# NVlabs/STEP

Hardware: NVIDIA H100
Metric: clips/sec (T=32,224x224) STEP max_iter=3 (higher is better)
Workload: dtype f16

## Files before the change

step_b200/csrc/conv_umma.cu:

```cuda
#include <cuda.h>
#include <stdlib.h>
#include <string.h>

#include "common.cuh"
#include "umma_ptx.cuh"

namespace step {

constexpr int kBM = 128;
constexpr int kMaxBN = 256;
constexpr int kStages = 8;
constexpr int kThreads = 384;
constexpr int kConsumers = 256;
constexpr int kCopyThreads = 96;
constexpr int kPersistMaxKBlocks = 100;
constexpr int kBookBytes = 2 * kStages * 8 + 2 * 8 + 2 * 2 * kMaxBN * 4;
constexpr int kProducerRegs = 40, kConsumerRegs = 232;

#define STEP_CONV_TILES(X)                                                                                         \
  X(64, 32) X(64, 64) X(64, 128) X(64, 144) X(64, 152) X(64, 176) X(64, 192) X(64, 208) X(64, 224) X(64, 256)      \
  X(32, 64) X(32, 128) X(32, 144) X(32, 152) X(32, 160) X(32, 208) X(32, 224)                                      \
  X(16, 64)

__host__ __device__ constexpr int staging_pitch(int BN) { return ((BN / 8 + 1) | 1) * 16; }

struct ConvGeom {
  int mode;
  int taps, KT, KH, KW, PT, PH, PW;
  int kblocks_per_tap;
  int BN, n_tiles;
  int n_stages;
  int n_splits, split[2], ld_extra[2], coff_extra[2];
  __half* y_extra[2];
  int Cout, out_ld, out_coff, res_ld, res_coff, relu;
  int OT, OH, OW, Nimg;
  long long M;
  int tiles;
  int bw, bh, bt, tiles_w, tiles_h, tiles_t;
  int a_bytes;
};

__device__ __forceinline__ long long tile_row_pixel(const ConvGeom& g, int m_tile, int row) {
  if (g.mode == STEP_A_BOX) {
    int r = m_tile;
    const int bw0 = (r % g.tiles_w) * g.bw; r /= g.tiles_w;
    const int bh0 = (r % g.tiles_h) * g.bh; r /= g.tiles_h;
    const int bt0 = (r % g.tiles_t) * g.bt; const int bn = r / g.tiles_t;
    const int dw = row % g.bw, rr = row / g.bw;
    const int dh = rr % g.bh, dt = rr / g.bh;
    const int ow = bw0 + dw, oh = bh0 + dh, ot = bt0 + dt;
    if (dt < g.bt && ow < g.OW && oh < g.OH && ot < g.OT) return (((long long)bn * g.OT + ot) * g.OH + oh) * g.OW + ow;
    return -1;
  }
  const long long m = (long long)m_tile * kBM + row;
  return m < g.M ? m : -1;
}

__device__ __forceinline__ bool mbar_try_wait(uint64_t* bar, uint32_t parity) {
  uint32_t done;
  asm volatile("{\n\t.reg .pred p;\n\tmbarrier.try_wait.parity.shared::cta.b64 p, [%1], %2;\n\tselp.u32 %0, 1, 0, p;\n\t}"
               : "=r"(done) : "r"(smem_u32(bar)), "r"(parity) : "memory");
  return done != 0;
}

template <int BK, int BN>
__global__ void __launch_bounds__(kThreads, 1)
conv_umma_kernel(const __grid_constant__ CUtensorMap map_a, const __grid_constant__ CUtensorMap map_b, ConvGeom g,
                 const float* __restrict__ scale, const float* __restrict__ shift, const __half* __restrict__ residual,
                 __half* __restrict__ y) {
  static_assert(BN % 8 == 0 && BN <= kMaxBN, "wgmma N is a multiple of 8, at most 256");
  constexpr bool kRealloc = BN > 128;
  constexpr bool kBulkOut = BN > 128;
  constexpr int kABytes = kBM * BK * 2;
  constexpr int kBBytes = BN * BK * 2;
  extern __shared__ __align__(1024) uint8_t smem_raw[];
  uint64_t* full_bar = (uint64_t*)smem_raw;
  uint64_t* empty_bar = full_bar + kStages;
  uint64_t* out_full = empty_bar + kStages;
  uint64_t* out_empty = out_full + 1;
  float* s_consts = (float*)(out_empty + 1);
  uint8_t* smem = (uint8_t*)(((uintptr_t)smem_raw + kBookBytes + 1023) & ~(uintptr_t)1023);
  uint8_t* sA = smem;
  uint8_t* sB = smem + g.n_stages * kABytes;
  uint8_t* stg = smem + g.n_stages * (kABytes + kBBytes);
  constexpr int pitch = staging_pitch(BN);

  const int warp = threadIdx.x >> 5, lane = threadIdx.x & 31;
  const int num_kb = g.taps * g.kblocks_per_tap;

  if (threadIdx.x == 0) {
    prefetch_tensormap(&map_a);
    prefetch_tensormap(&map_b);
    for (int s = 0; s < kStages; ++s) { mbar_init(&full_bar[s], 1); mbar_init(&empty_bar[s], 2); }
    mbar_init(out_full, kConsumers / 32);
    mbar_init(out_empty, kCopyThreads / 32);
    fence_barrier_init();
  }
  auto stage_consts = [&](int n_tile, int buf, int t, int nthr) {
    float* s_scale = s_consts + buf * 2 * kMaxBN;
    float* s_shift = s_scale + kMaxBN;
    for (int i = t; i < BN; i += nthr) {
      const int c = n_tile * BN + i;
      s_scale[i] = (scale && c < g.Cout) ? scale[c] : 1.0f;
      s_shift[i] = (shift && c < g.Cout) ? shift[c] : 0.0f;
    }
  };
  if (threadIdx.x < 128) stage_consts(blockIdx.x % g.n_tiles, 0, threadIdx.x, 128);
  __syncthreads();

  if (warp < 4) {
    if constexpr (kRealloc) setmaxnreg_dec<kProducerRegs>();
    if (warp == 0) {
      if (elect_one()) {
        const uint32_t tx_bytes = (uint32_t)(g.a_bytes + kBBytes);
        int stage = 0; uint32_t phase = 0;
        for (int tile = blockIdx.x; tile < g.tiles; tile += gridDim.x) {
          const int m_tile = tile / g.n_tiles, n0 = (tile - m_tile * g.n_tiles) * BN;
          long long m0 = (long long)m_tile * kBM;
          int bn = 0, bt0 = 0, bh0 = 0, bw0 = 0;
          if (g.mode == STEP_A_BOX) {
            int r = m_tile;
            bw0 = (r % g.tiles_w) * g.bw; r /= g.tiles_w;
            bh0 = (r % g.tiles_h) * g.bh; r /= g.tiles_h;
            bt0 = (r % g.tiles_t) * g.bt; bn = r / g.tiles_t;
          }
          int iw = 0, ih = 0, it = 0, in_ = 0;
          if (g.mode == STEP_A_IM2COL) {
            long long r = m0;
            iw = (int)(r % g.OW); r /= g.OW;
            ih = (int)(r % g.OH); r /= g.OH;
            it = (int)(r % g.OT); in_ = (int)(r / g.OT);
            iw -= g.PW; ih -= g.PH; it -= g.PT;
          }
          int kw = 0, kh = 0, kt = 0;
          for (int tap = 0; tap < g.taps; ++tap) {
            for (int kc = 0; kc < g.kblocks_per_tap; ++kc) {
              mbar_wait(&empty_bar[stage], phase ^ 1);
              mbar_expect_tx(&full_bar[stage], tx_bytes);
              const int c0 = kc * BK;
              uint8_t* a_dst = sA + stage * kABytes;
              if (g.mode == STEP_A_LINEAR) {
                tma_load_2d(&map_a, &full_bar[stage], a_dst, c0, (int)m0);
              } else if (g.mode == STEP_A_BOX) {
                tma_load_5d(&map_a, &full_bar[stage], a_dst, c0, bw0 + kw - g.PW, bh0 + kh - g.PH, bt0 + kt - g.PT, bn);
              } else {
                tma_load_im2col_5d(&map_a, &full_bar[stage], a_dst, c0, iw, ih, it, in_, (uint16_t)kw, (uint16_t)kh,
                                   (uint16_t)kt);
              }
              tma_load_3d(&map_b, &full_bar[stage], sB + stage * kBBytes, c0, tap, n0);
              if (++stage == g.n_stages) { stage = 0; phase ^= 1; }
            }
            if (++kw == g.KW) { kw = 0; if (++kh == g.KH) { kh = 0; ++kt; } }
          }
        }
      }
    } else {
      const int ct = threadIdx.x - 32;
      int i_tile = 0;
      for (int tile = blockIdx.x; tile < g.tiles; tile += gridDim.x, ++i_tile) {
        const int m_tile = tile / g.n_tiles, n0 = (tile - m_tile * g.n_tiles) * BN;
        if (tile + (int)gridDim.x < g.tiles) stage_consts((tile + gridDim.x) % g.n_tiles, (i_tile + 1) & 1, ct, kCopyThreads);
        while (!mbar_try_wait(out_full, i_tile & 1)) __nanosleep(128);
        if constexpr (!kBulkOut) {
          constexpr int cpr = BN / 8;
          constexpr int kUnroll = 4;
          for (int i0 = ct; i0 < kBM * cpr; i0 += kUnroll * kCopyThreads) {
            uint4 val[kUnroll];
#pragma unroll
            for (int u = 0; u < kUnroll; ++u) {
              const int i = i0 + u * kCopyThreads, rr = i / cpr, ch = i - rr * cpr;
              if (i < kBM * cpr) val[u] = *reinterpret_cast<const uint4*>(stg + (size_t)rr * pitch + ch * 16);
            }
#pragma unroll
            for (int u = 0; u < kUnroll; ++u) {
              const int i = i0 + u * kCopyThreads, rr = i / cpr, ch = i - rr * cpr;
              const int col = n0 + ch * 8;
              if (i >= kBM * cpr || col >= g.Cout) continue;
              const long long rp = tile_row_pixel(g, m_tile, rr);
              if (rp < 0) continue;
              __half* dst = y + (size_t)rp * g.out_ld + g.out_coff + col;
              if (g.n_splits > 0 && col >= g.split[0]) {
                const int d = (g.n_splits > 1 && col >= g.split[1]) ? 1 : 0;
                dst = g.y_extra[d] + (size_t)rp * g.ld_extra[d] + g.coff_extra[d] + (col - g.split[d]);
              }
              *reinterpret_cast<uint4*>(dst) = val[u];
            }
          }
          __syncwarp();
          if (lane == 0) mbar_arrive(out_empty);
          continue;
        }
        const int end = min(n0 + BN, g.Cout);
        for (int rr = ct; rr < kBM; rr += kCopyThreads) {
          const long long rp = tile_row_pixel(g, m_tile, rr);
          if (rp < 0) continue;
          for (int col = n0; col < end;) {
            __half* dst = y + (size_t)rp * g.out_ld + g.out_coff + col;
            int next = end;
            if (g.n_splits > 0) {
              if (col >= g.split[0]) {
                const int d = (g.n_splits > 1 && col >= g.split[1]) ? 1 : 0;
                dst = g.y_extra[d] + (size_t)rp * g.ld_extra[d] + g.coff_extra[d] + (col - g.split[d]);
                if (d == 0 && g.n_splits > 1) next = min(end, g.split[1]);
              } else {
                next = min(end, g.split[0]);
              }
            }
            bulk_store(dst, stg + (size_t)rr * pitch + (col - n0) * 2, (uint32_t)(next - col) * 2);
            col = next;
          }
        }
        bulk_commit();
        bulk_wait_read<0>();
        __syncwarp();
        if (lane == 0) mbar_arrive(out_empty);
      }
    }
  } else {
    if constexpr (kRealloc) setmaxnreg_inc<kConsumerRegs>();
    const int wg = (warp >> 2) - 1;
    const int ct = threadIdx.x - 128;
    const uint64_t hi = desc_hi_kmajor<BK>();
    const uint64_t a_lo0 = desc_lo(sA + wg * 64 * BK * 2), b_lo0 = desc_lo(sB);
    const int wrow = wg * 64 + (warp & 3) * 16 + (lane >> 2);
    float acc[BN / 2];
    int stage = 0; uint32_t phase = 0;
    int i_tile = 0;
    for (int tile = blockIdx.x; tile < g.tiles; tile += gridDim.x, ++i_tile) {
      const int m_tile = tile / g.n_tiles, n0 = (tile - m_tile * g.n_tiles) * BN;
#pragma unroll
      for (int i = 0; i < BN / 2; ++i) acc[i] = 0.0f;
      int prev = -1;
      for (int kb = 0; kb < num_kb; ++kb) {
        mbar_wait(&full_bar[stage], phase);
        const uint64_t a_lo = a_lo0 + (uint64_t)(stage * (kABytes >> 4)), b_lo = b_lo0 + (uint64_t)(stage * (kBBytes >> 4));
        wg_fence();
#pragma unroll
        for (int k = 0; k < BK / 16; ++k)
          wgmma_f16<BN>(acc, hi | (a_lo + 2 * k), hi | (b_lo + 2 * k), 1u);
        wg_commit();
        wg_wait<1>();
        if (prev >= 0 && ct % 128 == 0) mbar_arrive(&empty_bar[prev]);
        prev = stage;
        if (++stage == g.n_stages) { stage = 0; phase ^= 1; }
      }
      wg_wait<0>();
      if (ct % 128 == 0) mbar_arrive(&empty_bar[prev]);
      mbar_wait(out_empty, (i_tile & 1) ^ 1);
      const float* s_scale = s_consts + (i_tile & 1) * 2 * kMaxBN;
      const float* s_shift = s_scale + kMaxBN;
#pragma unroll
      for (int i = 0; i < 2; ++i) {
        const int row = wrow + 8 * i;
        const long long pix = residual ? tile_row_pixel(g, m_tile, row) : -1;
        const __half* rrow = pix >= 0 ? residual + (size_t)pix * g.res_ld + g.res_coff + n0 : nullptr;
        uint8_t* srow = stg + (size_t)row * pitch;
#pragma unroll
        for (int j = 0; j < BN / 8; ++j) {
          const int col = 8 * j + 2 * (lane & 3);
          float f0 = fmaf(acc[4 * j + 2 * i], s_scale[col], s_shift[col]);
          float f1 = fmaf(acc[4 * j + 2 * i + 1], s_scale[col + 1], s_shift[col + 1]);
          if (rrow && n0 + col < g.Cout) {
            const float2 rf = __half22float2(*reinterpret_cast<const __half2*>(rrow + col));
            f0 += rf.x; f1 += rf.y;
          }
          if (g.relu) { f0 = fmaxf(f0, 0.0f); f1 = fmaxf(f1, 0.0f); }
          *reinterpret_cast<__half2*>(srow + col * 2) = __floats2half2_rn(f0, f1);
        }
      }
      if constexpr (kBulkOut) fence_proxy_async();
      __syncwarp();
      if (lane == 0) mbar_arrive(out_full);
    }
  }
}

template <int BK>
__global__ void __launch_bounds__(32) tma_dump_kernel(const __grid_constant__ CUtensorMap map_a, ConvGeom g, int m_tile,
                                                      int kt, int kh, int kw, int c0, uint8_t* __restrict__ out) {
  constexpr int kABytes = kBM * BK * 2;
  extern __shared__ __align__(1024) uint8_t smem_raw[];
  uint8_t* smem = (uint8_t*)(((uintptr_t)smem_raw + 1023) & ~(uintptr_t)1023);
  __shared__ uint64_t bar;
  for (int i = threadIdx.x; i < kABytes / 4; i += 32) ((uint32_t*)smem)[i] = 0xFFFFFFFFu;
  if (threadIdx.x == 0) { mbar_init(&bar, 1); fence_barrier_init(); }
  fence_proxy_async();
  __syncwarp();
  if (threadIdx.x == 0) {
    long long m0 = (long long)m_tile * kBM;
    mbar_expect_tx(&bar, (uint32_t)g.a_bytes);
    if (g.mode == STEP_A_LINEAR) {
      tma_load_2d(&map_a, &bar, smem, c0, (int)m0);
    } else if (g.mode == STEP_A_BOX) {
      int r = m_tile;
      int bw0 = (r % g.tiles_w) * g.bw; r /= g.tiles_w;
      int bh0 = (r % g.tiles_h) * g.bh; r /= g.tiles_h;
      int bt0 = (r % g.tiles_t) * g.bt; int bn = r / g.tiles_t;
      tma_load_5d(&map_a, &bar, smem, c0, bw0 + kw - g.PW, bh0 + kh - g.PH, bt0 + kt - g.PT, bn);
    } else {
      long long r = m0;
      int iw = (int)(r % g.OW); r /= g.OW;
      int ih = (int)(r % g.OH); r /= g.OH;
      int it = (int)(r % g.OT); int in_ = (int)(r / g.OT);
      tma_load_im2col_5d(&map_a, &bar, smem, c0, iw - g.PW, ih - g.PH, it - g.PT, in_, (uint16_t)kw, (uint16_t)kh, (uint16_t)kt);
    }
  }
  mbar_wait(&bar, 0);
  __syncwarp();
  for (int i = threadIdx.x; i < kABytes / 4; i += 32) ((uint32_t*)out)[i] = ((uint32_t*)smem)[i];
}

static int pick_bk(int Cin) {
  if (Cin <= 16) return 16;
  const int k64 = (Cin + 63) / 64 * 64, k32 = (Cin + 31) / 32 * 32;
  return k32 < k64 ? 32 : 64;
}

struct ConvTile {
  int BK, BN;
  void (*kernel)(CUtensorMap, CUtensorMap, ConvGeom, const float*, const float*, const __half*, __half*);
};
static const ConvTile kTiles[] = {
#define STEP_TILE_ENTRY(bk, bn) {bk, bn, conv_umma_kernel<bk, bn>},
    STEP_CONV_TILES(STEP_TILE_ENTRY)
#undef STEP_TILE_ENTRY
};
constexpr int kNumTiles = (int)(sizeof(kTiles) / sizeof(kTiles[0]));

static int pick_tile(int BK, int Cout) {
  int best = -1; long best_pad = 0, best_n = 0;
  for (int i = 0; i < kNumTiles; ++i) {
    if (kTiles[i].BK != BK) continue;
    const long n = (Cout + kTiles[i].BN - 1) / kTiles[i].BN, pad = n * kTiles[i].BN - Cout;
    if (best < 0 || pad < best_pad || (pad == best_pad && n < best_n)) { best = i; best_pad = pad; best_n = n; }
  }
  return best;
}

static void pick_box(int OW, int OH, int OT, int* bw, int* bh, int* bt) {
  double best = -1;
  for (int w = 1; w <= OW && w <= kBM; ++w)
    for (int h = 1; h <= OH && w * h <= kBM; ++h) {
      int t = kBM / (w * h);
      if (t > OT) t = OT;
      if (t < 1) continue;
      double eff = ((double)OW / (((OW + w - 1) / w) * w)) * ((double)OH / (((OH + h - 1) / h) * h)) *
                   ((double)OT / (((OT + t - 1) / t) * t)) * ((double)(w * h * t) / kBM);
      if (eff > best + 1e-9) { best = eff; *bw = w; *bh = h; *bt = t; }
    }
}

static std::atomic<int> g_two_ctas[kNumTiles];
static std::atomic<unsigned long long> g_attr_seen[kNumTiles];

static int two_ctas_fit(int t, size_t smem, bool* two) {
  int v = g_two_ctas[t].load(std::memory_order_relaxed);
  if (v == 0) {
    cudaError_t e = cudaFuncSetAttribute(kTiles[t].kernel, cudaFuncAttributeMaxDynamicSharedMemorySize, 227 * 1024);
    int n = 0;
    if (e == cudaSuccess) e = cudaOccupancyMaxActiveBlocksPerMultiprocessor(&n, kTiles[t].kernel, kThreads, smem);
    if (e != cudaSuccess) { cudaGetLastError(); return fail((int)e, "conv3d(f16): occupancy query: %s", cudaGetErrorString(e)); }
    v = n >= 2 ? 2 : 1;
    g_two_ctas[t].store(v, std::memory_order_relaxed);
  }
  *two = v == 2;
  return 0;
}

static std::atomic<int> g_sm_count[64];

static int sm_count(int* n) {
  int dev = 0;
  cudaError_t e = cudaGetDevice(&dev);
  if (e != cudaSuccess) { cudaGetLastError(); return fail((int)e, "conv3d(f16): cudaGetDevice: %s", cudaGetErrorString(e)); }
  int v = g_sm_count[dev & 63].load(std::memory_order_relaxed);
  if (v == 0) {
    e = cudaDeviceGetAttribute(&v, cudaDevAttrMultiProcessorCount, dev);
    if (e != cudaSuccess) { cudaGetLastError(); return fail((int)e, "conv3d(f16): SM count: %s", cudaGetErrorString(e)); }
    g_sm_count[dev & 63].store(v, std::memory_order_relaxed);
  }
  *n = v;
  return 0;
}

struct ConvPlan {
  CUtensorMap map_a, map_b;
  ConvGeom g;
  int BK;
  int tile;
  size_t smem_bytes;
  dim3 grid;
};

static int build_plan(const step_conv_params* p, ConvPlan* pl) {
  STEP_CHECK_ARG(p->ST == 1 && p->SH == 1 && p->SW == 1, "conv3d(f16): stride must be 1 (use the s2d stem)");
  STEP_CHECK_ARG(p->Cin % 8 == 0 && p->in_ld % 8 == 0 && p->w_ld % 8 == 0 && p->w_ld >= p->Cin,
                 "conv3d(f16): Cin=%d in_ld=%d w_ld=%d must be multiples of 8", p->Cin, p->in_ld, p->w_ld);
  STEP_CHECK_ARG(p->Cout % 8 == 0 && p->out_ld % 8 == 0 && p->out_coff % 8 == 0, "conv3d(f16): Cout/out_ld/out_coff %% 8");
  STEP_CHECK_ARG(!p->residual || (p->res_ld % 8 == 0 && p->res_coff % 8 == 0), "conv3d(f16): res_ld/res_coff %% 8");
  STEP_CHECK_ARG((((uintptr_t)p->x | (uintptr_t)p->w | (uintptr_t)p->y | (uintptr_t)p->residual) & 15) == 0,
                 "conv3d(f16): pointers must be 16-byte aligned");
  ConvGeom& g = pl->g;
  memset(&g, 0, sizeof(g));
  const int taps = p->KT * p->KH * p->KW;
  const bool is_1x1 = taps == 1 && p->PT == 0 && p->PH == 0 && p->PW == 0 && p->OT == p->T && p->OH == p->H && p->OW == p->W;
  int mode = p->a_mode;
  if (mode == STEP_A_AUTO) mode = is_1x1 ? STEP_A_LINEAR : STEP_A_BOX;
  STEP_CHECK_ARG(mode == STEP_A_LINEAR || mode == STEP_A_BOX || mode == STEP_A_IM2COL, "conv3d(f16): bad a_mode %d", p->a_mode);
  STEP_CHECK_ARG(mode != STEP_A_LINEAR || is_1x1, "conv3d(f16): LINEAR mode needs a 1x1x1 unpadded filter");
  g.mode = mode;
  g.taps = taps; g.KT = p->KT; g.KH = p->KH; g.KW = p->KW; g.PT = p->PT; g.PH = p->PH; g.PW = p->PW;
  pl->BK = pick_bk(p->Cin);
  const int BK = pl->BK;
  g.kblocks_per_tap = (p->Cin + BK - 1) / BK;
  pl->tile = pick_tile(BK, p->Cout);
  g.BN = kTiles[pl->tile].BN;
  g.n_tiles = (p->Cout + g.BN - 1) / g.BN;
  g.Cout = p->Cout; g.out_ld = p->out_ld; g.out_coff = p->out_coff; g.res_ld = p->res_ld; g.res_coff = p->res_coff;
  g.relu = p->relu;
  g.n_splits = p->n_splits;
  if (p->n_splits) {
    STEP_CHECK_ARG(p->n_splits >= 1 && p->n_splits <= 2 && !p->residual, "conv3d(f16): fused outputs need no residual, 1-2 splits");
    int prev = 0;
    for (int i = 0; i < p->n_splits; ++i) {
      STEP_CHECK_ARG(p->split[i] % 16 == 0 && p->split[i] > prev && p->split[i] < p->Cout && p->y_extra[i] &&
                     p->ld_extra[i] % 8 == 0 && p->coff_extra[i] % 8 == 0 && ((uintptr_t)p->y_extra[i] & 15) == 0,
                     "conv3d(f16): bad split %d", i);
      prev = p->split[i];
      g.split[i] = p->split[i]; g.y_extra[i] = (__half*)p->y_extra[i]; g.ld_extra[i] = p->ld_extra[i]; g.coff_extra[i] = p->coff_extra[i];
    }
    STEP_CHECK_ARG(p->out_ld >= p->out_coff + p->split[0], "conv3d(f16): first destination too narrow");
  }
  g.OT = p->OT; g.OH = p->OH; g.OW = p->OW; g.Nimg = p->N;
  g.M = (long long)p->N * p->OT * p->OH * p->OW;
  long long m_tiles;
  int rc;
  if (mode == STEP_A_LINEAR) {
    STEP_CHECK_ARG(g.M < (1LL << 31), "conv3d(f16): M too large");
    rc = encode_rows2d(&pl->map_a, p->x, g.M, p->Cin, p->in_ld, BK, kBM, swizzle_for(BK), CU_TENSOR_MAP_L2_PROMOTION_L2_128B,
                       "conv3d(f16): A (linear)");
    m_tiles = (g.M + kBM - 1) / kBM;
    g.a_bytes = kBM * BK * 2;
  } else {
    const ActLayout act(p->N, p->T, p->H, p->W, p->Cin, p->in_ld);
    if (mode == STEP_A_BOX) {
      pick_box(p->OW, p->OH, p->OT, &g.bw, &g.bh, &g.bt);
      g.tiles_w = (p->OW + g.bw - 1) / g.bw; g.tiles_h = (p->OH + g.bh - 1) / g.bh; g.tiles_t = (p->OT + g.bt - 1) / g.bt;
      const cuuint32_t box[5] = {(cuuint32_t)BK, (cuuint32_t)g.bw, (cuuint32_t)g.bh, (cuuint32_t)g.bt, 1};
      rc = encode_act5d(&pl->map_a, p->x, act, box, swizzle_for(BK), CU_TENSOR_MAP_L2_PROMOTION_L2_128B, "conv3d(f16): A (box)");
      m_tiles = (long long)p->N * g.tiles_t * g.tiles_h * g.tiles_w;
      g.a_bytes = g.bw * g.bh * g.bt * BK * 2;
    } else {
      const int ph_t = p->OT - p->T + p->KT - 1 - p->PT, ph_h = p->OH - p->H + p->KH - 1 - p->PH,
                ph_w = p->OW - p->W + p->KW - 1 - p->PW;
      int lower[3] = {-p->PW, -p->PH, -p->PT};
      int upper[3] = {ph_w - (p->KW - 1), ph_h - (p->KH - 1), ph_t - (p->KT - 1)};
      for (int i = 0; i < 3; ++i)
        STEP_CHECK_ARG(lower[i] >= -16 && lower[i] <= 15 && upper[i] >= -16 && upper[i] <= 15, "conv3d(f16): im2col corner range");
      rc = encode_act5d_im2col(&pl->map_a, p->x, act, lower, upper, BK, kBM, swizzle_for(BK),
                               CU_TENSOR_MAP_L2_PROMOTION_L2_128B, "conv3d(f16): A (im2col)");
      int drv = 0;
      cudaDriverGetVersion(&drv);
      if (rc == 0 && drv <= 13010 &&
          (size_t)p->N * p->T * p->H * p->W * p->in_ld * 2 < 131072)
        reinterpret_cast<uint64_t*>(&pl->map_a)[1] &= ~(1ULL << 21);
      m_tiles = (g.M + kBM - 1) / kBM;
      g.a_bytes = kBM * BK * 2;
    }
  }
  if (rc) return rc;
  if ((rc = encode_weights3d(&pl->map_b, p->w, p->Cout, taps, p->Cin, p->w_ld, BK, g.BN, swizzle_for(BK),
                             CU_TENSOR_MAP_L2_PROMOTION_L2_256B, "conv3d(f16): B")))
    return rc;
  STEP_CHECK_ARG(m_tiles * g.n_tiles < (1LL << 31), "conv3d(f16): grid too large");
  g.tiles = (int)(m_tiles * g.n_tiles);
  const long per_stage = (long)kBM * BK * 2 + (long)g.BN * BK * 2;
  const long fixed = kBookBytes + 1024 + (long)kBM * staging_pitch(g.BN);
  int st = (int)((113L * 1024 - fixed) / per_stage);
  if (st > kStages) st = kStages;
  bool two = false;
  if (st >= 3) {
    if (int rc = two_ctas_fit(pl->tile, (size_t)(fixed + st * per_stage), &two)) return rc;
  }
  if (!two) st = (int)((227L * 1024 - fixed) / per_stage);
  g.n_stages = st > kStages ? kStages : st;
  STEP_CHECK_ARG(g.n_stages >= 2, "conv3d(f16): tile does not fit shared memory");
  pl->smem_bytes = (size_t)(fixed + g.n_stages * per_stage);
  int sms = 0;
  if (int rc = sm_count(&sms)) return rc;
  const long resident = (long)sms * (two ? 2 : 1);
  const bool persist = g.taps * g.kblocks_per_tap <= kPersistMaxKBlocks && g.tiles > resident;
  pl->grid = dim3((unsigned)(persist ? resident : g.tiles));
  return 0;
}

int conv3d_umma_launch(const step_conv_params* p, step_stream_t stream) {
  ConvPlan pl;
  if (int rc = build_plan(p, &pl)) return rc;
  const ConvTile& t = kTiles[pl.tile];
  if (int rc = allow_dynamic_smem(t.kernel, g_attr_seen[pl.tile], 227 * 1024, "conv_umma_kernel")) return rc;
  return launch_tc("conv_umma_kernel", t.kernel, pl.grid, kThreads, pl.smem_bytes, cu(stream), pl.map_a, pl.map_b, pl.g,
                   p->scale, p->shift, (const __half*)p->residual, (__half*)p->y);
}

}

using namespace step;

extern "C" int step_debug_tma_tile(const step_conv_params* p, int m_tile, int kt, int kh, int kw, int c0, void* out,
                                   int* bk_out, int* box_out , step_stream_t stream) {
  ConvPlan pl;
  if (int rc = build_plan(p, &pl)) return rc;
  if (bk_out) *bk_out = pl.BK;
  if (box_out) { box_out[0] = pl.g.bw; box_out[1] = pl.g.bh; box_out[2] = pl.g.bt; }
  size_t smem = 1024 + (size_t)kBM * pl.BK * 2;
  if (pl.BK == 64) tma_dump_kernel<64><<<1, 32, smem, cu(stream)>>>(pl.map_a, pl.g, m_tile, kt, kh, kw, c0, (uint8_t*)out);
  else if (pl.BK == 32) tma_dump_kernel<32><<<1, 32, smem, cu(stream)>>>(pl.map_a, pl.g, m_tile, kt, kh, kw, c0, (uint8_t*)out);
  else tma_dump_kernel<16><<<1, 32, smem, cu(stream)>>>(pl.map_a, pl.g, m_tile, kt, kh, kw, c0, (uint8_t*)out);
  STEP_LAUNCH_CHECK("tma_dump_kernel");
  return 0;
}
```

Baseline: 1161.

## Load and multiply only the needed channels in the last K block

Adds narrower tail tensor maps for activations and weights so the last K block of each tap loads only the channels it needs (16, 32 or 64 wide). The consumer runs fewer wgmma K-steps for that block, using a matching descriptor and per-warpgroup offset. BK selection now weighs N-tile padding for BK 64 against BK 32, and several BK=32 tile variants are dropped. This removes zero-padding traffic and MMA work when Cin is not a multiple of BK, at the cost of extra tensor maps, more kernel parameters and more template branching.

```diff
diff --git a/step_b200/csrc/conv_umma.cu b/step_b200/csrc/conv_umma.cu
--- a/step_b200/csrc/conv_umma.cu
+++ b/step_b200/csrc/conv_umma.cu
@@ -1,6 +1,8 @@
 #include <cuda.h>
 #include <stdlib.h>
 #include <string.h>
+
+#include <type_traits>
 
 #include "common.cuh"
 #include "umma_ptx.cuh"
@@ -19,8 +21,13 @@
 
 #define STEP_CONV_TILES(X)                                                                                         \
   X(64, 32) X(64, 64) X(64, 128) X(64, 144) X(64, 152) X(64, 176) X(64, 192) X(64, 208) X(64, 224) X(64, 256)      \
-  X(32, 64) X(32, 128) X(32, 144) X(32, 152) X(32, 160) X(32, 208) X(32, 224)                                      \
+  X(32, 64) X(32, 128) X(32, 160)                                                                                  \
   X(16, 64)
+
+__host__ __device__ constexpr int tail_width(int tail, int BK) {
+  const int w = tail <= 1 ? 16 : (tail == 2 ? 32 : 64);
+  return w < BK ? w : BK;
+}
 
 __host__ __device__ constexpr int staging_pitch(int BN) { return ((BN / 8 + 1) | 1) * 16; }
 
@@ -28,6 +35,8 @@
   int mode;
   int taps, KT, KH, KW, PT, PH, PW;
   int kblocks_per_tap;
+  int tail;
+  int tail_w, a_tail_bytes;
   int BN, n_tiles;
   int n_stages;
   int n_splits, split[2], ld_extra[2], coff_extra[2];
@@ -65,7 +74,8 @@
 
 template <int BK, int BN>
 __global__ void __launch_bounds__(kThreads, 1)
-conv_umma_kernel(const __grid_constant__ CUtensorMap map_a, const __grid_constant__ CUtensorMap map_b, ConvGeom g,
+conv_umma_kernel(const __grid_constant__ CUtensorMap map_a, const __grid_constant__ CUtensorMap map_b,
+                 const __grid_constant__ CUtensorMap map_a_tail, const __grid_constant__ CUtensorMap map_b_tail, ConvGeom g,
                  const float* __restrict__ scale, const float* __restrict__ shift, const __half* __restrict__ residual,
                  __half* __restrict__ y) {
   static_assert(BN % 8 == 0 && BN <= kMaxBN, "wgmma N is a multiple of 8, at most 256");
@@ -86,11 +96,11 @@
   constexpr int pitch = staging_pitch(BN);
 
   const int warp = threadIdx.x >> 5, lane = threadIdx.x & 31;
-  const int num_kb = g.taps * g.kblocks_per_tap;
 
   if (threadIdx.x == 0) {
     prefetch_tensormap(&map_a);
     prefetch_tensormap(&map_b);
+    if (g.tail_w < BK) { prefetch_tensormap(&map_a_tail); prefetch_tensormap(&map_b_tail); }
     for (int s = 0; s < kStages; ++s) { mbar_init(&full_bar[s], 1); mbar_init(&empty_bar[s], 2); }
     mbar_init(out_full, kConsumers / 32);
     mbar_init(out_empty, kCopyThreads / 32);
@@ -113,6 +123,7 @@
     if (warp == 0) {
       if (elect_one()) {
         const uint32_t tx_bytes = (uint32_t)(g.a_bytes + kBBytes);
+        const uint32_t tx_tail = (uint32_t)(g.a_tail_bytes + BN * g.tail_w * 2);
         int stage = 0; uint32_t phase = 0;
         for (int tile = blockIdx.x; tile < g.tiles; tile += gridDim.x) {
           const int m_tile = tile / g.n_tiles, n0 = (tile - m_tile * g.n_tiles) * BN;
@@ -135,19 +146,21 @@
           int kw = 0, kh = 0, kt = 0;
           for (int tap = 0; tap < g.taps; ++tap) {
             for (int kc = 0; kc < g.kblocks_per_tap; ++kc) {
+              const bool narrow = kc == g.kblocks_per_tap - 1 && g.tail_w < BK;
+              const CUtensorMap* ma = narrow ? &map_a_tail : &map_a;
               mbar_wait(&empty_bar[stage], phase ^ 1);
-              mbar_expect_tx(&full_bar[stage], tx_bytes);
+              mbar_expect_tx(&full_bar[stage], narrow ? tx_tail : tx_bytes);
               const int c0 = kc * BK;
               uint8_t* a_dst = sA + stage * kABytes;
               if (g.mode == STEP_A_LINEAR) {
-                tma_load_2d(&map_a, &full_bar[stage], a_dst, c0, (int)m0);
+                tma_load_2d(ma, &full_bar[stage], a_dst, c0, (int)m0);
               } else if (g.mode == STEP_A_BOX) {
-                tma_load_5d(&map_a, &full_bar[stage], a_dst, c0, bw0 + kw - g.PW, bh0 + kh - g.PH, bt0 + kt - g.PT, bn);
+                tma_load_5d(ma, &full_bar[stage], a_dst, c0, bw0 + kw - g.PW, bh0 + kh - g.PH, bt0 + kt - g.PT, bn);
               } else {
-                tma_load_im2col_5d(&map_a, &full_bar[stage], a_dst, c0, iw, ih, it, in_, (uint16_t)kw, (uint16_t)kh,
+                tma_load_im2col_5d(ma, &full_bar[stage], a_dst, c0, iw, ih, it, in_, (uint16_t)kw, (uint16_t)kh,
                                    (uint16_t)kt);
               }
-              tma_load_3d(&map_b, &full_bar[stage], sB + stage * kBBytes, c0, tap, n0);
+              tma_load_3d(narrow ? &map_b_tail : &map_b, &full_bar[stage], sB + stage * kBBytes, c0, tap, n0);
               if (++stage == g.n_stages) { stage = 0; phase ^= 1; }
             }
             if (++kw == g.KW) { kw = 0; if (++kh == g.KH) { kh = 0; ++kt; } }
@@ -220,8 +233,7 @@
     if constexpr (kRealloc) setmaxnreg_inc<kConsumerRegs>();
     const int wg = (warp >> 2) - 1;
     const int ct = threadIdx.x - 128;
-    const uint64_t hi = desc_hi_kmajor<BK>();
-    const uint64_t a_lo0 = desc_lo(sA + wg * 64 * BK * 2), b_lo0 = desc_lo(sB);
+    const uint64_t a_lo0 = desc_lo(sA), b_lo0 = desc_lo(sB);
     const int wrow = wg * 64 + (warp & 3) * 16 + (lane >> 2);
     float acc[BN / 2];
     int stage = 0; uint32_t phase = 0;
@@ -231,18 +243,40 @@
 #pragma unroll
       for (int i = 0; i < BN / 2; ++i) acc[i] = 0.0f;
       int prev = -1;
-      for (int kb = 0; kb < num_kb; ++kb) {
+      auto kblock = [&](auto steps, auto width) {
+        const uint64_t hi = desc_hi_kmajor<decltype(width)::value>();
         mbar_wait(&full_bar[stage], phase);
-        const uint64_t a_lo = a_lo0 + (uint64_t)(stage * (kABytes >> 4)), b_lo = b_lo0 + (uint64_t)(stage * (kBBytes >> 4));
+        constexpr int wg_rows = (64 * decltype(width)::value * 2) >> 4;
+        const uint64_t a_lo = a_lo0 + (uint64_t)(stage * (kABytes >> 4) + wg * wg_rows);
+        const uint64_t b_lo = b_lo0 + (uint64_t)(stage * (kBBytes >> 4));
         wg_fence();
 #pragma unroll
-        for (int k = 0; k < BK / 16; ++k)
+        for (int k = 0; k < decltype(steps)::value; ++k)
           wgmma_f16<BN>(acc, hi | (a_lo + 2 * k), hi | (b_lo + 2 * k), 1u);
         wg_commit();
         wg_wait<1>();
         if (prev >= 0 && ct % 128 == 0) mbar_arrive(&empty_bar[prev]);
         prev = stage;
         if (++stage == g.n_stages) { stage = 0; phase ^= 1; }
+      };
+      using full = std::integral_constant<int, BK / 16>;
+      using bk = std::integral_constant<int, BK>;
+      for (int tap = 0; tap < g.taps; ++tap) {
+        for (int kc = 1; kc < g.kblocks_per_tap; ++kc) kblock(full(), bk());
+        switch (g.tail) {
+          case 1:
+            kblock(std::integral_constant<int, 1>(), std::integral_constant<int, tail_width(1, BK)>());
+            break;
+          case 2:
+            kblock(std::integral_constant<int, 2 < BK / 16 ? 2 : BK / 16>(), std::integral_constant<int, tail_width(2, BK)>());
+            break;
+          case 3:
+            kblock(std::integral_constant<int, 3 < BK / 16 ? 3 : BK / 16>(), std::integral_constant<int, tail_width(3, BK)>());
+            break;
+          default:
+            kblock(full(), bk());
+            break;
+        }
       }
       wg_wait<0>();
       if (ct % 128 == 0) mbar_arrive(&empty_bar[prev]);
@@ -310,15 +344,10 @@
   for (int i = threadIdx.x; i < kABytes / 4; i += 32) ((uint32_t*)out)[i] = ((uint32_t*)smem)[i];
 }
 
-static int pick_bk(int Cin) {
-  if (Cin <= 16) return 16;
-  const int k64 = (Cin + 63) / 64 * 64, k32 = (Cin + 31) / 32 * 32;
-  return k32 < k64 ? 32 : 64;
-}
-
 struct ConvTile {
   int BK, BN;
-  void (*kernel)(CUtensorMap, CUtensorMap, ConvGeom, const float*, const float*, const __half*, __half*);
+  void (*kernel)(CUtensorMap, CUtensorMap, CUtensorMap, CUtensorMap, ConvGeom, const float*, const float*, const __half*,
+                 __half*);
 };
 static const ConvTile kTiles[] = {
 #define STEP_TILE_ENTRY(bk, bn) {bk, bn, conv_umma_kernel<bk, bn>},
@@ -335,6 +364,17 @@
     if (best < 0 || pad < best_pad || (pad == best_pad && n < best_n)) { best = i; best_pad = pad; best_n = n; }
   }
   return best;
+}
+
+static int pick_tile_bk(int Cin, int Cout, int* BK) {
+  if (Cin <= 32) { *BK = Cin <= 16 ? 16 : 32; return pick_tile(*BK, Cout); }
+  const int t64 = pick_tile(64, Cout), t32 = pick_tile(32, Cout);
+  auto cost = [&](int t, long* n) { *n = (Cout + kTiles[t].BN - 1) / kTiles[t].BN; return *n * kTiles[t].BN - Cout; };
+  long n64, n32;
+  const long pad64 = cost(t64, &n64), pad32 = cost(t32, &n32);
+  const bool narrow = pad32 < pad64 || (pad32 == pad64 && n32 < n64);
+  *BK = narrow ? 32 : 64;
+  return narrow ? t32 : t64;
 }
 
 static void pick_box(int OW, int OH, int OT, int* bw, int* bh, int* bt) {
@@ -385,6 +425,7 @@
 
 struct ConvPlan {
   CUtensorMap map_a, map_b;
+  CUtensorMap map_a_tail, map_b_tail;
   ConvGeom g;
   int BK;
   int tile;
@@ -410,10 +451,12 @@
   STEP_CHECK_ARG(mode != STEP_A_LINEAR || is_1x1, "conv3d(f16): LINEAR mode needs a 1x1x1 unpadded filter");
   g.mode = mode;
   g.taps = taps; g.KT = p->KT; g.KH = p->KH; g.KW = p->KW; g.PT = p->PT; g.PH = p->PH; g.PW = p->PW;
-  pl->BK = pick_bk(p->Cin);
+  pl->tile = pick_tile_bk(p->Cin, p->Cout, &pl->BK);
   const int BK = pl->BK;
   g.kblocks_per_tap = (p->Cin + BK - 1) / BK;
-  pl->tile = pick_tile(BK, p->Cout);
+  g.tail = (p->Cin - (g.kblocks_per_tap - 1) * BK + 15) / 16;
+  g.tail_w = tail_width(g.tail, BK);
+  const int TW = g.tail_w;
   g.BN = kTiles[pl->tile].BN;
   g.n_tiles = (p->Cout + g.BN - 1) / g.BN;
   g.Cout = p->Cout; g.out_ld = p->out_ld; g.out_coff = p->out_coff; g.res_ld = p->res_ld; g.res_coff = p->res_coff;
@@ -439,8 +482,12 @@
     STEP_CHECK_ARG(g.M < (1LL << 31), "conv3d(f16): M too large");
     rc = encode_rows2d(&pl->map_a, p->x, g.M, p->Cin, p->in_ld, BK, kBM, swizzle_for(BK), CU_TENSOR_MAP_L2_PROMOTION_L2_128B,
                        "conv3d(f16): A (linear)");
+    if (rc == 0 && TW < BK)
+      rc = encode_rows2d(&pl->map_a_tail, p->x, g.M, p->Cin, p->in_ld, TW, kBM, swizzle_for(TW),
+                         CU_TENSOR_MAP_L2_PROMOTION_L2_128B, "conv3d(f16): A tail (linear)");
     m_tiles = (g.M + kBM - 1) / kBM;
     g.a_bytes = kBM * BK * 2;
+    g.a_tail_bytes = kBM * TW * 2;
   } else {
     const ActLayout act(p->N, p->T, p->H, p->W, p->Cin, p->in_ld);
     if (mode == STEP_A_BOX) {
@@ -448,8 +495,13 @@
       g.tiles_w = (p->OW + g.bw - 1) / g.bw; g.tiles_h = (p->OH + g.bh - 1) / g.bh; g.tiles_t = (p->OT + g.bt - 1) / g.bt;
       const cuuint32_t box[5] = {(cuuint32_t)BK, (cuuint32_t)g.bw, (cuuint32_t)g.bh, (cuuint32_t)g.bt, 1};
       rc = encode_act5d(&pl->map_a, p->x, act, box, swizzle_for(BK), CU_TENSOR_MAP_L2_PROMOTION_L2_128B, "conv3d(f16): A (box)");
+      const cuuint32_t box_tail[5] = {(cuuint32_t)TW, (cuuint32_t)g.bw, (cuuint32_t)g.bh, (cuuint32_t)g.bt, 1};
+      if (rc == 0 && TW < BK)
+        rc = encode_act5d(&pl->map_a_tail, p->x, act, box_tail, swizzle_for(TW), CU_TENSOR_MAP_L2_PROMOTION_L2_128B,
+                          "conv3d(f16): A tail (box)");
       m_tiles = (long long)p->N * g.tiles_t * g.tiles_h * g.tiles_w;
       g.a_bytes = g.bw * g.bh * g.bt * BK * 2;
+      g.a_tail_bytes = g.bw * g.bh * g.bt * TW * 2;
     } else {
       const int ph_t = p->OT - p->T + p->KT - 1 - p->PT, ph_h = p->OH - p->H + p->KH - 1 - p->PH,
                 ph_w = p->OW - p->W + p->KW - 1 - p->PW;
@@ -459,19 +511,33 @@
         STEP_CHECK_ARG(lower[i] >= -16 && lower[i] <= 15 && upper[i] >= -16 && upper[i] <= 15, "conv3d(f16): im2col corner range");
       rc = encode_act5d_im2col(&pl->map_a, p->x, act, lower, upper, BK, kBM, swizzle_for(BK),
                                CU_TENSOR_MAP_L2_PROMOTION_L2_128B, "conv3d(f16): A (im2col)");
+      if (rc == 0 && TW < BK)
+        rc = encode_act5d_im2col(&pl->map_a_tail, p->x, act, lower, upper, TW, kBM, swizzle_for(TW),
+                                 CU_TENSOR_MAP_L2_PROMOTION_L2_128B, "conv3d(f16): A tail (im2col)");
       int drv = 0;
       cudaDriverGetVersion(&drv);
       if (rc == 0 && drv <= 13010 &&
-          (size_t)p->N * p->T * p->H * p->W * p->in_ld * 2 < 131072)
+          (size_t)p->N * p->T * p->H * p->W * p->in_ld * 2 < 131072) {
         reinterpret_cast<uint64_t*>(&pl->map_a)[1] &= ~(1ULL << 21);
+        if (TW < BK) reinterpret_cast<uint64_t*>(&pl->map_a_tail)[1] &= ~(1ULL << 21);
+      }
       m_tiles = (g.M + kBM - 1) / kBM;
       g.a_bytes = kBM * BK * 2;
+      g.a_tail_bytes = kBM * TW * 2;
     }
   }
   if (rc) return rc;
   if ((rc = encode_weights3d(&pl->map_b, p->w, p->Cout, taps, p->Cin, p->w_ld, BK, g.BN, swizzle_for(BK),
                              CU_TENSOR_MAP_L2_PROMOTION_L2_256B, "conv3d(f16): B")))
     return rc;
+  if (TW < BK) {
+    if ((rc = encode_weights3d(&pl->map_b_tail, p->w, p->Cout, taps, p->Cin, p->w_ld, TW, g.BN, swizzle_for(TW),
+                               CU_TENSOR_MAP_L2_PROMOTION_L2_256B, "conv3d(f16): B tail")))
+      return rc;
+  } else {
+    pl->map_a_tail = pl->map_a;
+    pl->map_b_tail = pl->map_b;
+  }
   STEP_CHECK_ARG(m_tiles * g.n_tiles < (1LL << 31), "conv3d(f16): grid too large");
   g.tiles = (int)(m_tiles * g.n_tiles);
   const long per_stage = (long)kBM * BK * 2 + (long)g.BN * BK * 2;
@@ -499,8 +565,8 @@
   if (int rc = build_plan(p, &pl)) return rc;
   const ConvTile& t = kTiles[pl.tile];
   if (int rc = allow_dynamic_smem(t.kernel, g_attr_seen[pl.tile], 227 * 1024, "conv_umma_kernel")) return rc;
-  return launch_tc("conv_umma_kernel", t.kernel, pl.grid, kThreads, pl.smem_bytes, cu(stream), pl.map_a, pl.map_b, pl.g,
-                   p->scale, p->shift, (const __half*)p->residual, (__half*)p->y);
+  return launch_tc("conv_umma_kernel", t.kernel, pl.grid, kThreads, pl.smem_bytes, cu(stream), pl.map_a, pl.map_b,
+                   pl.map_a_tail, pl.map_b_tail, pl.g, p->scale, p->shift, (const __half*)p->residual, (__half*)p->y);
 }
 
 }
```

Result: no change. 1162 (median of 6 runs) (+0.0%).
